# lemerleau/RAFFT

Measured on AMD Instinct MI355X. Metric: sequences/sec (whole node) on benchmark set, beam N=100; kcal/mol MAE vs CPU, higher is better.
Workload: dtype f32 FFT -> exact int counts, f64 scores, i32 dcal energies

## Files before the change

### rafft_amd/csrc/rafft_expand_small.hip

```cpp
#pragma once

template <int TL> struct SmLds {
    static constexpr int NL = 2 * TL;
    static constexpr int off_S = 0;
    static constexpr int off_pos = SM_SPAN + 8;
    static constexpr int off_br = off_pos + 2 * TL;
    static constexpr int off_pe = off_br + 4 * TL;
    static constexpr int off_psp = off_pe + 8 * (TL + 1);
    static constexpr int off_ck = (off_psp + 2 * (TL + 1) + 7) & ~7;
    static constexpr int off_val = off_ck + 8 * NL;
    static constexpr int per_team = (off_val + 8 * NL + 15) & ~15;
};
#define SM_GUARD 4608
static_assert(sizeof(SmallT) <= SM_GUARD, "energy tables must fit the guard area");
#define SM_WG_WAVES 4
template <int TL> constexpr int small_lds_bytes() { return SM_GUARD + SM_WG_WAVES * (64 / TL) * SmLds<TL>::per_team; }

#ifndef RAFFT_SMALL_WAVES
#define RAFFT_SMALL_WAVES 4
#endif

__device__ __forceinline__ uint32_t sm_shift(uint32_t x, int s)
{
    return s >= 0 ? (s < 32 ? x >> s : 0u) : (s > -32 ? x << -s : 0u);
}

template <int TL, bool PROD = false>
__global__ __launch_bounds__(64 * SM_WG_WAVES, RAFFT_SMALL_WAVES) void expand_small_kernel(Dev d, int cls_arg)
{
    const int cls = cls_arg & 0xFF;
    using LY = SmLds<TL>;
    constexpr int TPW = 64 / TL;
    extern __shared__ __align__(16) unsigned char lds_all[];
    {
        int *dst = (int *)lds_all;
        const int *src = (const int *)&d.T->s;
        for (int i = threadIdx.x; i < (int)(sizeof(SmallT) / 4); i += 64 * SM_WG_WAVES) dst[i] = src[i];
        __syncthreads();
    }
    const SmallT *T = (const SmallT *)lds_all;
    const BigT *B = &d.T->b;
    const int lane = threadIdx.x & 63, wv = threadIdx.x >> 6;
    const int tl = lane & (TL - 1), tq = lane / TL, tbase = tq * TL;
    const unsigned long long tmask = ((1ULL << TL) - 1ULL) << tbase;
    const unsigned long long lt_lane = (1ULL << lane) - 1ULL, lt_team = (1ULL << tbase) - 1ULL;
    const uint32_t TM = (uint32_t)((1ULL << TL) - 1ULL);
    unsigned char *lds = lds_all + SM_GUARD + (wv * TPW + tq) * LY::per_team;
    uint8_t *Sw = lds + LY::off_S;
    uint16_t *pos = (uint16_t *)(lds + LY::off_pos);
    uint32_t *brl = (uint32_t *)(lds + LY::off_br);
    int *pe_ext = (int *)(lds + LY::off_pe), *pe_ml = pe_ext + (TL + 1);
    uint16_t *psp = (uint16_t *)(lds + LY::off_psp);
    unsigned long long *ck = (unsigned long long *)(lds + LY::off_ck);
    double *val = (double *)(lds + LY::off_val);

    if (d.c->overflow) return;
    const unsigned n_items = d.c->n_work[cls].v;
    const unsigned gw = blockIdx.x * SM_WG_WAVES + wv, n_waves = gridDim.x * SM_WG_WAVES;
    if (gw == 0 && lane == 0) d.c->n_mat = 0;
    const int shard = gw & (NSHARD - 1);
    unsigned long long st_items = 0, st_n = 0, st_lags = 0, st_nbr = 0;
    unsigned int st_eval = 0, st_guess = 0, st_kguess = 0;
    const unsigned FETCH = n_items > 4u * TPW * n_waves ? (unsigned)d.fetch_bulk : 1u;
    unsigned fetch_base = 0, fetch_left = 0;
    const FetchPlan fplan = fetch_plan(d, n_items, FETCH * TPW, TPW);
    int fshard = (int)(gw & (NSHARD - 1));
    unsigned long long ffailed = 0;
    unsigned long long slab_base = 0; unsigned slab_left = 0;
    const bool dbg = !PROD && d.dbg.lag != nullptr;
    const double par_none = 0.0; (void)par_none;

    for (;;) {
        wave_sync();
        if (fetch_left == 0) {
            unsigned fcount = TPW;
            fetch_base = fetch_chunk(d, cls, fplan, fshard, ffailed, fcount);
            if (fetch_base == ~0u) break;
            fetch_left = fcount / TPW;
        }
        const unsigned item0 = fetch_base;
        fetch_base += TPW; fetch_left--;
        if (item0 >= n_items) { fetch_left = 0; continue; }
        const bool act = item0 + (unsigned)tq < n_items;
        const int nid = d.work[cls][act ? item0 + tq : item0];
        const NodeRec *nr = &d.nd[nid];
        const int n = nr->n, ci = nr->ci, cj = nr->cj, nbr = nr->nbr, L = nr->L, par_dcal = nr->pdcal;
        const uint16_t *posg = d.pos + nr->pos;
        const uint32_t *brg = d.br + nr->br;
        const uint8_t *codes = d.codes + nr->soff;
        const int sx0 = ci < 0 ? 0 : ci;
        const uint8_t *Sl = (const uint8_t *)Sw - sx0;
        const int m = 2 * n - 1;

        int myp = -1, c = 0;
        if (act && tl < n) {
            const int p = posg[tl];
            myp = p & 0x0FFF; c = p >> 12;
            pos[tl] = (uint16_t)myp;
            Sw[myp - sx0] = (uint8_t)c;
        }
        if (act && tl < nbr) {
            const uint32_t u = brg[tl];
            brl[tl] = u & 0x0FFF0FFFu;
            Sw[(int)(u & 0x0FFFu) - sx0] = (uint8_t)((u >> 12) & 0xFu);
            Sw[(int)((u >> 16) & 0x0FFFu) - sx0] = (uint8_t)(u >> 28);
        }
        if (act && ci >= 0 && tl < 2) { const int x = tl ? cj : ci; Sw[x - sx0] = codes[x]; }
        const uint32_t px_ = row16_or((uint32_t)((c + 3) & 3) << (2 * (tl & 15)));
        const unsigned long long p2 = (unsigned long long)(uint32_t)__shfl((int)px_, tbase + 15, 64) |
                                      (TL == 32 ? (unsigned long long)(uint32_t)__shfl((int)px_, tbase + 31, 64) << 32 : 0ULL);
        const unsigned long long bA = __ballot(c == 1), bC = __ballot(c == 2), bG = __ballot(c == 3), bU = __ballot(c == 4);
        const int pprev = __shfl_up(myp, 1, TL);
        const unsigned long long bg = __ballot(act && tl >= 1 && tl < n && myp - pprev == 1);
        const uint32_t mA = (uint32_t)(bA >> tbase) & TM, mC = (uint32_t)(bC >> tbase) & TM, mG = (uint32_t)(bG >> tbase) & TM,
                       mU = (uint32_t)(bU >> tbase) & TM, mg = (uint32_t)(bg >> tbase) & TM;
        const int rs = 32 - n;
        const uint32_t rA = __brev(mA) >> rs, rC = __brev(mC) >> rs, rG = __brev(mG) >> rs, rU = __brev(mU) >> rs, rg = __brev(mg) >> rs;
        wave_sync();
        double wgc = d.gc, wau = d.au, wgu = d.gu;
        asm volatile("" : "+v"(wgc), "+v"(wau), "+v"(wgu));

        int w_nb[2], w_mi[2], w_mj[2];
        double w_sc[2];
#pragma unroll
        for (int s = 0; s < 2; s++) {
            const int k = tl + s * TL;
            int mx_nb = 0, mx_i = 0, mx_j = 0;
            double mx_s = 0.0;
            if (act && k < m) {
                const int len = k < n ? k + 1 : 2 * n - k - 1;
                const int len2 = (len >> 1) + (len & 1);
                const int ip0 = k < n ? 0 : k - n + 1, jp0 = k < n ? k : n - 1;
                const int csure = len - 1 - d.min_hp;
                int lo = csure > 0 ? min((csure + 1) >> 1, len2) : 0, hi = len2;
                while (lo < hi) {
                    const int mid = (lo + hi) >> 1;
                    if ((int)pos[jp0 - mid] - (int)pos[ip0 + mid] > d.min_hp) lo = mid + 1; else hi = mid;
                }
                const int lim = lo;
                if (lim > 0) {
                    const int sft = n - 1 - k;
                    const uint32_t xA = sm_shift(rA, sft), xC = sm_shift(rC, sft), xG = sm_shift(rG, sft), xU = sm_shift(rU, sft);
                    const uint32_t pGC = d.gc != 0.0 ? ((mG & xC) | (mC & xG)) : 0u;
                    const uint32_t pAU = d.au != 0.0 ? ((mA & xU) | (mU & xA)) : 0u;
                    const uint32_t pGU = d.gu != 0.0 ? ((mG & xU) | (mU & xG)) : 0u;
                    const uint32_t cm = mg & sm_shift(rg, sft - 1) & ~(1u << ip0);
                    const uint32_t range = (lim >= 32 ? ~0u : ((1u << lim) - 1u)) << ip0;
                    uint32_t any = (pGC | pAU | pGU) & range;
                    double prev = 0.0;
                    int last_ip = -2, runlen = 0;
                    bool found = false;
                    while (any) {
                        const int ip = __ffs((int)any) - 1;
                        any &= any - 1;
                        const uint32_t bit = 1u << ip;
                        const double w8 = (pGC & bit) ? wgc : (pAU & bit) ? wau : wgu;
                        if (ip != last_ip + 1) { prev = 0.0; runlen = 0; }
                        double t = w8;
                        if (cm & bit) t = (prev + w8) * w8;
                        runlen++;
                        if (t >= mx_s) { mx_s = t; mx_nb = runlen; mx_i = ip; mx_j = k - ip; found = true; }
                        prev = t; last_ip = ip;
                    }
                    if (!found) { mx_i = ip0 + lim - 1; mx_j = k - mx_i; }
                }
            }
            w_nb[s] = mx_nb; w_mi[s] = mx_i; w_mj[s] = mx_j; w_sc[s] = mx_s;
        }

        int w_k[2] = {tl, tl + TL};
        if (!dbg) {
            const unsigned long long sb0 = __ballot(w_nb[0] > 0) & tmask, sb1 = __ballot(w_nb[1] > 0) & tmask;
            const int n0 = __popcll(sb0), nst = n0 + __popcll(sb1);
            uint32_t *sl = (uint32_t *)ck;
            if (w_nb[0] > 0) sl[__popcll(sb0 & lt_lane)] = (uint32_t)w_nb[0] | ((uint32_t)w_mi[0] << 8) | ((uint32_t)tl << 16);
            if (w_nb[1] > 0) sl[n0 + __popcll(sb1 & lt_lane)] = (uint32_t)w_nb[1] | ((uint32_t)w_mi[1] << 8) | ((uint32_t)(tl + TL) << 16);
            wave_sync();
#pragma unroll
            for (int s = 0; s < 2; s++) {
                const int idx = tl + s * TL;
                const uint32_t e = idx < nst ? sl[idx] : 0u;
                w_nb[s] = (int)(e & 255u); w_mi[s] = (int)((e >> 8) & 255u); w_k[s] = (int)(e >> 16); w_mj[s] = w_k[s] - w_mi[s];
            }
            wave_sync();
        }
        {
            int ve = 0, vm = 0, vs = 0;
            if (act && tl < nbr) {
                const uint32_t u = brl[tl];
                const int p = (int)(u & 0xffffu), q = (int)(u >> 16);
                const int tt = pair_type(Sl[p], Sl[q]);
                if (ci < 0) ve = e_stem(T, tt, p > 0 ? (int)Sl[p - 1] : -1, q < L - 1 ? (int)Sl[q + 1] : -1, true);
                vm = e_stem(T, tt, p > 0 ? (int)Sl[p - 1] : 0, q < L - 1 ? (int)Sl[q + 1] : 0, false);
                vs = q - p + 1;
            }
            int xe = ve, xm = vm, xs = vs;
#pragma unroll
            for (int o = 1; o < TL; o <<= 1) {
                const int ye = __shfl_up(xe, o, TL), ym = __shfl_up(xm, o, TL), ys = __shfl_up(xs, o, TL);
                if (tl >= o) { xe += ye; xm += ym; xs += ys; }
            }
            if (act && tl < nbr) { pe_ext[tl] = xe - ve; pe_ml[tl] = xm - vm; psp[tl] = (uint16_t)(xs - vs); }
            if (act && tl == (nbr > 0 ? nbr - 1 : 0)) {
                if (nbr > 0) { pe_ext[nbr] = xe; pe_ml[nbr] = xm; psp[nbr] = (uint16_t)xs; }
                else { pe_ext[0] = 0; pe_ml[0] = 0; psp[0] = 0; }
            }
        }
        wave_sync();
        const double par_e = dcal_to_energy(par_dcal);
        const BrPrefix pf{pe_ext, pe_ml, psp};
        int w_dd[2];
        bool w_keep[2];
        {
            const bool anystem = act && (w_nb[0] > 0 || w_nb[1] > 0);
            int e_old = 0, g_old = 0;
            if (anystem) {
                const BrList all_br{brl, 0, nbr, 0, 0, 0, 0, 0};
                e_old = loop_energy_pre(T, B, Sl, L, ci, cj, all_br, pf, g_old);
            }
#pragma unroll
            for (int s = 0; s < 2; s++) {
                w_dd[s] = 0; w_keep[s] = false;
                const int nb = w_nb[s];
                if (act && nb > 0) {
                    int g = g_old;
                    const int mi = w_mi[s], mj = w_mj[s];
                    const int a0 = pos[mi], b0 = pos[mj], ao = pos[mi - nb + 1], bo = pos[mj + nb - 1];
                    int lo, hi, lo_o, hi_o;
                    br_lower4(brl, nbr, a0, b0, ao, bo, lo, hi, lo_o, hi_o);
                    BrList outer{brl, 0, lo_o, hi_o, nbr, 1, ao, bo};
                    int e_new = loop_energy_pre(T, B, Sl, L, ci, cj, outer, pf, g);
                    BrList inner{brl, lo, hi, 0, 0, 0, 0, 0};
                    e_new += loop_energy_pre(T, B, Sl, L, a0, b0, inner, pf, g);
                    if (nb <= 16 && a0 - ao == nb - 1 && bo - b0 == nb - 1)
                        e_new += stem_stack_windows(T, (uint32_t)(p2 >> (2 * (mi - nb + 1))), (uint32_t)(p2 >> (2 * mj)), nb);
                    else {
                    int pa = a0, pb = b0, ty_in = pair_type(Sl[a0], Sl[b0]);
                    for (int t = 1; t < nb; t++) {
                        const int a = pos[mi - t], b = pos[mj + t];
                        const int ty = pair_type(Sl[a], Sl[b]);
                        if (pa == a + 1 && pb == b - 1)
                            e_new += T->stack[ty][rtype(ty_in)];
                        else {
                            const int lo2 = br_lower(brl, nbr, a), hi2 = br_lower(brl, nbr, b);
                            BrList mid{brl, lo2, lo, hi, hi2, 1, pa, pb};
                            e_new += loop_energy_pre(T, B, Sl, L, a, b, mid, pf, g);
                            lo = lo2; hi = hi2;
                        }
                        pa = a; pb = b; ty_in = ty;
                    }
                    }
                    const int ddc = e_new - e_old;
                    w_dd[s] = ddc;
                    const double dE = dcal_to_energy(par_dcal + ddc) - par_e;
                    w_keep[s] = dE < d.min_nrj;
                    st_eval++; st_guess += g ? 1 : 0; st_kguess += (g && w_keep[s]) ? 1 : 0;
                }
            }
        }
        double w_val[2] = {0.0, 0.0};
#pragma unroll
        for (int s = 0; s < 2; s++) {
            const int k = w_k[s];
            if ((w_keep[s] || dbg) && act && k < m) {
                const int sft = n - 1 - k;
                const uint32_t xU = sm_shift(rU, sft), xC = sm_shift(rC, sft);
                const double nAU = 2.0 * (double)__popc(mA & xU), nGC = 2.0 * (double)__popc(mG & xC), nGU = 2.0 * (double)__popc(mG & xU);
                const double raw = nAU * d.au + nGC * d.gc + nGU * d.gu;
                const int nk = k < m - 1 - k ? k : m - 1 - k;
                w_val[s] = raw / ((double)nk + 1.0);
            }
        }
        int w_rank[2] = {0, 0};
        if (dbg) {
#pragma unroll
            for (int s = 0; s < 2; s++) { const int k = tl + s * TL; if (act && k < m) val[k] = w_val[s]; }
            wave_sync();
#pragma unroll
            for (int s = 0; s < 2; s++) {
                const int k = tl + s * TL;
                if (act && k < m && tq == 0) {
                    int r = 0;
                    for (int y = 0; y < m; y++) { const double v = val[y]; r += (v > w_val[s] || (v == w_val[s] && y > k)) ? 1 : 0; }
                    w_rank[s] = r;
                    d.dbg.lag[r] = k; d.dbg.corval[r] = w_val[s];
                    d.dbg.nb[r] = w_nb[s]; d.dbg.mi[r] = w_mi[s]; d.dbg.mj[r] = w_mj[s]; d.dbg.score[r] = w_sc[s];
                    if (d.dbg.ddcal) d.dbg.ddcal[r] = w_nb[s] > 0 ? w_dd[s] : INT_MIN;
                }
            }
            if (lane == 0 && d.dbg.n_ranked) *d.dbg.n_ranked = m;
            wave_sync();
        }

        const unsigned long long kb0 = __ballot(w_keep[0]), kb1 = __ballot(w_keep[1]);
        const int nk0 = __popcll(kb0 & tmask), nkept = nk0 + __popcll(kb1 & tmask);
        const int toff = __popcll(kb0 & lt_team) + __popcll(kb1 & lt_team);
        const int tot = __popcll(kb0) + __popcll(kb1);
        const int slot[2] = {(int)__popcll(kb0 & tmask & lt_lane), nk0 + (int)__popcll(kb1 & tmask & lt_lane)};
        unsigned long long cbase = 0;
        int ovf = 0;
        if (lane == 0 && tot) {
            if ((unsigned)tot > slab_left) {
                const unsigned slab = d.cand_shard_cap >= 64u * (unsigned)d.cand_slab ? (unsigned)d.cand_slab : 16u;
                const unsigned want = (unsigned)tot > slab ? (unsigned)tot : slab;
                const unsigned long long b0 = atomicAdd(&d.c->cand[shard].v, (unsigned long long)want);
                if (b0 + want > d.cand_shard_cap) { atomicOr(&d.c->overflow, OVF_CAND); ovf = 1; slab_left = 0; }
                else { slab_base = (unsigned long long)shard * d.cand_shard_cap + b0; slab_left = want; }
            }
            if (!ovf) { cbase = slab_base; slab_base += tot; slab_left -= tot; }
        }
        cbase = __shfl(cbase, 0, 64);
        ovf = __shfl(ovf, 0, 64);
#pragma unroll
        for (int s = 0; s < 2; s++)
            if (w_keep[s]) {
                ck[slot[s]] = ((unsigned long long)((unsigned)w_dd[s] ^ 0x80000000u) << 32) | (unsigned)w_k[s];
                val[slot[s]] = w_val[s];
            }
        wave_sync();
        if (!ovf) {
#pragma unroll
            for (int s = 0; s < 2; s++)
                if (w_keep[s]) {
                    const int k = w_k[s];
                    const unsigned long long kx = ck[slot[s]];
                    int rank = 0;
                    for (int y = 0; y < nkept; y++) {
                        const unsigned long long ky = ck[y];
                        if ((ky >> 32) == (kx >> 32)) {
                            const int lagq = (int)(ky & 0xFFFFFFFFu);
                            const double qv = val[y];
                            rank += (lagq != k && (qv > w_val[s] || (qv == w_val[s] && lagq > k))) ? 1 : 0;
                        } else
                            rank += ky < kx ? 1 : 0;
                    }
                    const int mi = w_mi[s], mj = w_mj[s], nb = w_nb[s];
                    const int a0 = pos[mi], b0 = pos[mj], ao = pos[mi - nb + 1], bo = pos[mj + nb - 1];
                    uint64_t h1 = 0, h2 = 0;
                    if (a0 - ao == nb - 1 && bo - b0 == nb - 1) stem_hash(a0, b0, ao, bo, &h1, &h2);
                    else
                        for (int t = 0; t < nb; t++) {
                            uint64_t a, b;
                            pair_hash(pos[mi - t], pos[mj + t], &a, &b);
                            h1 += a; h2 += b;
                        }
                    Cand cd;
                    cd.ddcal = w_dd[s]; cd.mi = (uint16_t)mi; cd.mj = (uint16_t)mj; cd.nb = (uint16_t)nb;
                    { int c0, c1, c2, c3; br_lower4(brl, nbr, a0, b0, ao, bo, c0, c1, c2, c3); cd.set_cuts(c0, c1, c2, c3); }
                    cd.h1 = h1; cd.h2 = h2;
                    d.cand[cbase + toff + rank] = cd;
                    d.cslot[cbase + toff + rank] = 0ULL;
                    if (dbg && d.dbg.kept) d.dbg.kept[rank] = w_rank[s];
                }
        }
        if (act && tl == 0) {
            NodeRec *nw = &d.nd[nid];
            nw->cand = cbase + toff;
            nw->ncand = ovf ? 0 : nkept;
            if (dbg && d.dbg.n_ranked) d.dbg.n_ranked[1] = nkept;
            st_items++; st_n += n; st_lags += m; st_nbr += nbr;
        }
    }
    for (int o = 32; o > 0; o >>= 1) {
        st_items += __shfl_xor(st_items, o, 64); st_n += __shfl_xor(st_n, o, 64);
        st_lags += __shfl_xor(st_lags, o, 64); st_nbr += __shfl_xor(st_nbr, o, 64);
        st_eval += __shfl_xor(st_eval, o, 64); st_guess += __shfl_xor(st_guess, o, 64); st_kguess += __shfl_xor(st_kguess, o, 64);
    }
    if (lane == 0 && st_items) {
        Counters::StatLine *sl = &d.c->xstat[cls][gw & (NSHARD - 1)];
        atomicAdd(&sl->items, st_items);
        atomicAdd(&sl->n, st_n);
        atomicAdd(&sl->lags, st_lags);
        atomicAdd(&sl->nbr, st_nbr);
        if (T->lsb && st_eval) {
            atomicAdd(&sl->evals, (unsigned long long)st_eval);
            if (st_guess) atomicAdd(&sl->guessed, (unsigned long long)st_guess);
            if (st_kguess) atomicAdd(&sl->kept_guessed, (unsigned long long)st_kguess);
        }
    }
}
```

### rafft_amd/csrc/rafft_kernels.hip

```cpp
#include "rafft_kernels.h"


__device__ __forceinline__ float2 cmul(float2 a, float2 b)
{
    return make_float2(a.x * b.x - a.y * b.y, a.x * b.y + a.y * b.x);
}
__device__ __forceinline__ float2 cmulc(float2 a, float2 b)
{
    return make_float2(a.x * b.x + a.y * b.y, a.y * b.x - a.x * b.y);
}

__device__ __forceinline__ void pin(unsigned int &x) { asm volatile("" : "+v"(x)); }
__device__ __forceinline__ void pin(int &x) { asm volatile("" : "+v"(x)); }
__device__ __forceinline__ void pin(unsigned long long &x) { asm volatile("" : "+v"(x)); }
__device__ __forceinline__ void pin(ulonglong2 &x) { asm volatile("" : "+v"(x.x), "+v"(x.y)); }
__device__ __forceinline__ void pin(uint4 &x) { asm volatile("" : "+v"(x.x), "+v"(x.y), "+v"(x.z), "+v"(x.w)); }

template <int NT>
__device__ inline int block_exscan(int v, int *scratch, int *tot)
{
    const int lane = threadIdx.x & 63, wv = threadIdx.x >> 6;
    const int x = wave_incl_scan(v);
    if (NT == 64) {
        *tot = __builtin_amdgcn_readlane(x, 63);
// ... 508 lines not shown
        }
        if (selected) {
            int *hist = (int *)(lds + lay.offA + (LONGSEQ == 2 ? lay.szA - 2048 : nofft ? 8 * P + 8 * MASK_WORDS * ((nmax + 63) >> 6) : 9 * P));
            int *shs = hist + 256;
            auto ukey = [&](int i) -> unsigned long long {
                unsigned long long u = (unsigned long long)__double_as_longlong(keyv[i]);
                return (u >> 63) ? ~u : (u | 0x8000000000000000ULL);
            };
            unsigned long long prefix = 0;
            int kk = Kp;
            bool take_ge = false;
            int pass0 = 7;
            if (PROD) {
                if (NT > 64) {
                    if (tid < 3) shs[20 + tid] = 0;
                    ESYNC();
                    if ((tid & 63) == 0) { atomicAdd(&shs[20], c_hi); atomicAdd(&shs[21], c_lo); atomicOr(&shs[22], c_odd); }
                    ESYNC();
                    c_hi = shs[20]; c_lo = shs[21]; c_odd = shs[22];
                }
                if (!c_odd) {
                    const int c_zero = m - c_hi - c_lo;
                    int binc;
                    if (kk <= c_hi) { prefix = 0xC0ULL << 56; binc = c_hi; }
                    else if (kk <= c_hi + c_lo) { prefix = 0xBFULL << 56; kk -= c_hi; binc = c_lo; }
                    else { prefix = 0x80ULL << 56; kk -= c_hi + c_lo; binc = c_zero; }
                    pass0 = kk == binc ? -1 : 6;
                    take_ge = kk == binc;
                }
            }
            for (int pass = pass0; pass >= 0; pass--) {
                for (int i = tid; i < 256; i += NT) hist[i] = 0;
                ESYNC();
                const int sh_hi = 8 * (pass + 1);
                for (int i = tid; i < m; i += NT) {
                    const unsigned long long u = ukey(i);
                    if (pass == 7 || (u >> sh_hi) == (prefix >> sh_hi)) atomicAdd(&hist[(int)((u >> (8 * pass)) & 255ULL)], 1);
                }
                ESYNC();
                {
                    constexpr int BPT = NT >= 256 ? 1 : 256 / NT;
                    int hs[BPT], mine = 0;
#pragma unroll
                    for (int j = 0; j < BPT; j++) { const int bi = tid * BPT + j; hs[j] = bi < 256 ? hist[255 - bi] : 0; mine += hs[j]; }
                    int tot, ex = block_exscan<NT>(mine, shs, &tot);
#pragma unroll
                    for (int j = 0; j < BPT; j++) {
                        if (ex < kk && kk <= ex + hs[j] && hs[j] > 0) { shs[28] = 255 - (tid * BPT + j); shs[29] = kk - ex; shs[30] = hs[j]; }
                        ex += hs[j];
                    }
                    ESYNC();
                }
                prefix |= (unsigned long long)(unsigned)shs[28] << (8 * pass);
                kk = shs[29];
                const bool whole_bin = kk == shs[30];
                ESYNC();
                if (whole_bin) { take_ge = true; break; }
            }
            int outn = 0, tie_run = 0;
            for (int base = 0; base < P; base += NT) {
                const int i = P - 1 - (base + tid);
                unsigned long long u = 0;
                int tie = 0;
                if (i >= 0 && i < m) { u = ukey(i); tie = (u == prefix) ? 1 : 0; }
                int ttot = 0, tex = 0;
                if (!take_ge) tex = block_exscan_flag<NT>(tie, shs, &ttot);
                const int g = (i >= 0 && i < m) && (take_ge ? u >= prefix : (u > prefix || (tie && tie_run + tex < kk))) ? 1 : 0;
                int gtot, gex = block_exscan_flag<NT>(g, shs, &gtot);
                if (g) rk[outn + gex] = (uint16_t)i;
                outn += gtot; tie_run += ttot;
                ESYNC();
            }
            if (dbgrank) {
            int M2 = 2; while (M2 < Kp) M2 <<= 1;
            for (int i = Kp + tid; i < M2; i += NT) rk[i] = 0xFFFF;
            ESYNC();
            for (int k2 = 2; k2 <= M2; k2 <<= 1)
                for (int j = k2 >> 1; j > 0; j >>= 1) {
                    for (int i = tid; i < M2; i += NT) {
                        int ixj = i ^ j;
                        if (ixj > i) {
                            const uint16_t la = rk[i], lb = rk[ixj];
                            bool a_first;
                            if (la == 0xFFFF) a_first = false;
                            else if (lb == 0xFFFF) a_first = true;
                            else { const double va = keyv[la], vb = keyv[lb]; a_first = (va > vb) || (va == vb && la > lb); }
                            const bool up = (i & k2) == 0;
                            if (up ? !a_first : a_first) { rk[i] = lb; rk[ixj] = la; }
                        }
                    }
                    ESYNC();
                }
            }
            for (int r = tid; r < Kp; r += NT)
                if (dbg.lag) { dbg.lag[r] = rk[r]; dbg.corval[r] = keyv[rk[r]]; }
            if (tid == 0 && dbg.n_ranked) *dbg.n_ranked = Kp;
            ESYNC();
        } else {
        if (inplace)
            for (int k2 = 2; k2 <= P; k2 <<= 1) {
                for (int j = k2 >> 1; j > 0; j >>= 1) {
                    for (int i = tid; i < P; i += NT) {
                        int ixj = i ^ j;
                        if (ixj > i) {
                            double va = keyv[i], vb = keyv[ixj];
                            uint16_t la = lagk[i], lb = lagk[ixj];
                            bool a_first = (va > vb) || (va == vb && la > lb);
                            bool up = (i & k2) == 0;
                            if (up ? !a_first : a_first) {
                                keyv[i] = vb; keyv[ixj] = va;
                                lagk[i] = lb; lagk[ixj] = la;
                            }
                        }
                    }
                    ESYNC();
                }
            }
        for (int r = tid; r < Kp; r += NT) {
            rk[r] = inplace ? lagk[r] : (uint16_t)r;
            if (dbg.lag) { dbg.lag[r] = lagk[r]; dbg.corval[r] = keyv[r]; }
        }
        if (tid == 0 && dbg.n_ranked) *dbg.n_ranked = Kp;
        ESYNC();
        }

        const int C = (NT >= 256 && selected) ? max(1, min(8, NT / max(Kp, 1))) : 1;
        struct WsPart { double score; int nb, mi, mj, any; };
        WsPart *parts = (WsPart *)(lds + lay.offA + 8 * Pk);
        const bool ws_masks = PROD || (d.gc >= 0.0 && d.au >= 0.0 && d.gu >= 0.0 && !force_fft);
        if (ws_masks) {
            const int W = (n + 63) >> 6;
            unsigned long long *F = (unsigned long long *)(lds + lay.offA + (inplace ? 0 : 8 * Pk));
            unsigned long long *R = F + MASK_F_WORDS * W;
            parts = (WsPart *)(R + 5 * W);
            if (LONGSEQ != 2 && (!mw || inplace)) {
                build_masks<NT>(F, R, W, n, code_at, pos, tid);
                ESYNC();
            }
            const uint32_t *F32 = (const uint32_t *)F, *R32 = (const uint32_t *)R;
            const int W2 = 2 * W;
            double wgc = d.gc, wau = d.au, wgu = d.gu;
            asm volatile("" : "+v"(wgc), "+v"(wau), "+v"(wgu));
            auto win = [](const uint32_t *X, int start) -> uint32_t { const int q_ = start >> 5; return __builtin_amdgcn_alignbit(X[q_ + 1], X[q_], (uint32_t)(start & 31)); };
            for (int q = tid; q < Kp * C; q += NT) {
                const int r = q / C, c = q - r * C;
                const int lagp = rk[r];
                const int len = lagp < n ? lagp + 1 : 2 * n - lagp - 1;
                const int len2 = (len >> 1) + (len & 1);
                const int ip0 = lagp < n ? 0 : lagp - n + 1, jp0 = lagp < n ? lagp : n - 1;
                const int csure = len - 1 - d.min_hp;
                int lo = csure > 0 ? min((csure + 1) >> 1, len2) : 0, hi = len2;
                while (lo < hi) {
                    const int mid = (lo + hi) >> 1;
                    if ((int)pos[jp0 - mid] - (int)pos[ip0 + mid] > d.min_hp) lo = mid + 1; else hi = mid;
                }
                const int lim = lo;
                const int ca = (int)((long long)lim * c / C), ce = (int)((long long)lim * (c + 1) / C);
                const int rs0 = n - 1 - lagp + ip0;
                auto cells = [&](int k, uint32_t &pGC, uint32_t &pAU, uint32_t &pGU, uint32_t &cm) {
                    const int cs = ip0 + 32 * k, rs = rs0 + 32 * k;
                    const uint32_t fA = win(F32 + 0 * W2, cs), fC = win(F32 + 1 * W2, cs), fG = win(F32 + 2 * W2, cs), fU = win(F32 + 3 * W2, cs);
                    const uint32_t xA = win(R32 + 0 * W2, rs), xC = win(R32 + 1 * W2, rs), xG = win(R32 + 2 * W2, rs), xU = win(R32 + 3 * W2, rs);
                    pGC = d.gc != 0.0 ? ((fG & xC) | (fC & xG)) : 0u;
                    pAU = d.au != 0.0 ? ((fA & xU) | (fU & xA)) : 0u;
                    pGU = d.gu != 0.0 ? ((fG & xU) | (fU & xG)) : 0u;
                    cm = win(F32 + 4 * W2, cs) & win(R32 + 4 * W2, rs);
                    if (k == 0) cm &= ~1u;
                };
                auto span = [](int lo_, int hi_, int cb) -> uint32_t {
                    uint32_t m_ = ~0u;
                    if (lo_ > cb) m_ &= ~0u << (lo_ - cb);
                    if (hi_ < cb + 32) m_ &= (1u << (hi_ - cb)) - 1u;
                    return m_;
                };
                double mx_s = 0.0, prev = 0.0;
                int mx_nb = 0, mx_c = 0, last_c = -2, runlen = 0, mx_i = 0, mx_j = 0;
                if (ce > ca) {
                    int z = ca;
                    if (ca > 0) {
                        for (int kz = (ca - 1) >> 5;; kz--) {
                            const int cb = kz << 5;
                            uint32_t pGC, pAU, pGU, cm;
                            cells(kz, pGC, pAU, pGU, cm);
                            const uint32_t zeros = ~(pGC | pAU | pGU) & span(0, ca, cb);
                            if (zeros) { z = cb + 32 - __clz((int)zeros); break; }
                            if (cb == 0) { z = 0; break; }
                        }
                    }
                    for (int k = z >> 5; k <= (ce - 1) >> 5; k++) {
                        const int cb = k << 5;
                        uint32_t pGC, pAU, pGU, cm;
                        cells(k, pGC, pAU, pGU, cm);
                        uint32_t any = (pGC | pAU | pGU) & span(z, ce, cb);
                        while (any) {
                            const int bi = __ffs((int)any) - 1;
                            any &= any - 1u;
                            const int cc = cb + bi;
                            const double w8 = ((pGC >> bi) & 1u) ? wgc : ((pAU >> bi) & 1u) ? wau : wgu;
                            if (cc != last_c + 1) { prev = 0.0; runlen = 0; }
                            double t = w8;
                            if ((cm >> bi) & 1u) t = (prev + w8) * w8;
                            runlen++;
                            if ((C == 1 || cc >= ca) && t >= mx_s) { mx_s = t; mx_nb = runlen; mx_c = cc; }
                            prev = t; last_c = cc;
                        }
                    }
                    if (mx_nb == 0) mx_c = ce - 1;
                    mx_i = ip0 + mx_c; mx_j = lagp - mx_i;
                }
                if (C == 1) {
                    wnb[r] = (uint16_t)mx_nb; wmi[r] = (uint16_t)mx_i;
                    if (dbg.nb) { dbg.nb[r] = mx_nb; dbg.mi[r] = mx_i; dbg.mj[r] = mx_j; dbg.score[r] = mx_s; }
                } else {
                    WsPart wp; wp.score = mx_s; wp.nb = mx_nb; wp.mi = mx_i; wp.mj = mx_j; wp.any = ce > ca ? 1 : 0;
                    parts[q] = wp;
                }
            }
            if (C > 1) {
                ESYNC();
                for (int r = tid; r < Kp; r += NT) {
                    double mx_s = 0.0;
                    int mx_nb = 0, mx_i = 0, mx_j = 0;
                    for (int c = 0; c < C; c++) {
                        const WsPart wp = parts[r * C + c];
                        if (wp.any && wp.score >= mx_s) { mx_s = wp.score; mx_nb = wp.nb; mx_i = wp.mi; mx_j = wp.mj; }
                    }
                    wnb[r] = (uint16_t)mx_nb; wmi[r] = (uint16_t)mx_i;
                    if (dbg.nb) { dbg.nb[r] = mx_nb; dbg.mi[r] = mx_i; dbg.mj[r] = mx_j; dbg.score[r] = mx_s; }
                }
            }
        } else {
            for (int q = tid; q < Kp * C; q += NT) {
                const int r = q / C, c = q - r * C;
                const int lagp = rk[r];
                const int len = lagp < n ? lagp + 1 : 2 * n - lagp - 1;
                const int len2 = (len >> 1) + (len & 1);
                const int a = (int)((long long)len2 * c / C), e = (int)((long long)len2 * (c + 1) / C);
                const int ip0 = lagp < n ? 0 : lagp - n + 1, jp0 = lagp < n ? lagp : n - 1;
                int z = a;
                while (z > 0 && wtab[code_at(ip0 + z - 1) * 5 + code_at(jp0 - (z - 1))] != 0.0) z--;
                double prev = 0.0, mx_s = 0.0;
                int tmp = 0, mx_nb = 0, mx_i = 0, mx_j = 0, any = 0;
                for (int i = z; i < e; i++) {
                    const int ip = ip0 + i, jp = jp0 - i;
                    double t = wtab[code_at(ip) * 5 + code_at(jp)];
                    if (i > 0 && (int)pos[ip] - (int)pos[ip - 1] == 1 && (int)pos[jp + 1] - (int)pos[jp] == 1)
                        t = (prev + t) * t;
                    tmp = (t == 0.0) ? 0 : tmp + 1;
                    if (i >= a && t >= mx_s && (int)pos[jp] - (int)pos[ip] > d.min_hp) {
                        mx_s = t; mx_nb = tmp; mx_i = ip; mx_j = jp; any = 1;
                    }
                    prev = t;
                }
                if (C == 1) {
                    wnb[r] = (uint16_t)mx_nb; wmi[r] = (uint16_t)mx_i;
                    if (dbg.nb) { dbg.nb[r] = mx_nb; dbg.mi[r] = mx_i; dbg.mj[r] = mx_j; dbg.score[r] = mx_s; }
                } else {
                    WsPart w; w.score = mx_s; w.nb = mx_nb; w.mi = mx_i; w.mj = mx_j; w.any = any;
                    parts[q] = w;
                }
            }
            if (C > 1) {
                ESYNC();
                for (int r = tid; r < Kp; r += NT) {
                    double mx_s = 0.0;
                    int mx_nb = 0, mx_i = 0, mx_j = 0;
                    for (int c = 0; c < C; c++) {
                        const WsPart w = parts[r * C + c];
                        if (w.any && w.score >= mx_s) { mx_s = w.score; mx_nb = w.nb; mx_i = w.mi; mx_j = w.mj; }
                    }
                    wnb[r] = (uint16_t)mx_nb; wmi[r] = (uint16_t)mx_i;
                    if (dbg.nb) { dbg.nb[r] = mx_nb; dbg.mi[r] = mx_i; dbg.mj[r] = mx_j; dbg.score[r] = mx_s; }
                }
            }
        }
        ESYNC();

        const double par_e = dcal_to_energy(par_dcal);
        int *pe_ext = (int *)(lds + lay.offA + (inplace ? 0 : 8 * Pk));
        int *pe_ml = pe_ext + (nbr + 1);
        uint16_t *psp = (uint16_t *)(pe_ml + (nbr + 1));
        if (tid < 64) {
            int c_e = 0, c_m = 0, c_s = 0;
            for (int base = 0; base < nbr; base += 64) {
                const int i = base + tid;
                int ve = 0, vm = 0, vs = 0;
                if (i < nbr) {
                    const uint32_t u = brl[i];
                    const int p = (int)(u & 0xffffu), q = (int)(u >> 16);
                    const int tt = pair_type(Sl[p], Sl[q]);
                    if (ci < 0) ve = e_stem(T, tt, p > 0 ? (int)Sl[p - 1] : -1, q < L - 1 ? (int)Sl[q + 1] : -1, true);
                    vm = e_stem(T, tt, p > 0 ? (int)Sl[p - 1] : 0, q < L - 1 ? (int)Sl[q + 1] : 0, false);
                    vs = q - p + 1;
                }
                const int xe = wave_incl_scan(ve), xm = wave_incl_scan(vm), xs = wave_incl_scan(vs);
                if (i < nbr) { pe_ext[i] = c_e + xe - ve; pe_ml[i] = c_m + xm - vm; psp[i] = (uint16_t)(c_s + xs - vs); }
                c_e += __builtin_amdgcn_readlane(xe, 63); c_m += __builtin_amdgcn_readlane(xm, 63); c_s += __builtin_amdgcn_readlane(xs, 63);
            }
            if (tid == 0) { pe_ext[nbr] = c_e; pe_ml[nbr] = c_m; psp[nbr] = (uint16_t)c_s; }
        }
        ESYNC();
        const BrPrefix pf{pe_ext, pe_ml, psp};
        const BrList all_br{brl, 0, nbr, 0, 0, 0, 0, 0};
        int g_old = 0;
        const int e_old = loop_energy_pre(T, B, Sl, L, ci, cj, all_br, pf, g_old);
        int nst = 0;
        for (int base = 0; base < Kp; base += NT) {
            const int r = base + tid;
            const int f = (r < Kp && wnb[r] > 0) ? 1 : 0;
            if (r < Kp) keep[r] = 0;
            int tot, ex = block_exscan_flag<NT>(f, misc + 16, &tot);
            if (f) widx[nst + ex] = (uint16_t)r;
            nst += tot;
        }
        ESYNC();
        for (int si = tid; si < nst; si += NT) {
            const int r = widx[si];
            const int nb = wnb[r];
            {
                int g = g_old;
                const int mi = wmi[r], mj = (int)rk[r] - mi;
                const int a0 = pos[mi], b0 = pos[mj], ao = pos[mi - nb + 1], bo = pos[mj + nb - 1];
                int lo, hi, lo_o, hi_o;
                br_lower4(brl, nbr, a0, b0, ao, bo, lo, hi, lo_o, hi_o);
                BrList outer{brl, 0, lo_o, hi_o, nbr, 1, ao, bo};
                int e_new = loop_energy_pre(T, B, Sl, L, ci, cj, outer, pf, g);
                BrList inner{brl, lo, hi, 0, 0, 0, 0, 0};
                e_new += loop_energy_pre(T, B, Sl, L, a0, b0, inner, pf, g);
                if (CODE_LDS && nb <= 16 && a0 - ao == nb - 1 && bo - b0 == nb - 1)
                    e_new += stem_stack_windows(T, strand_window(P2, mi - nb + 1), strand_window(P2, mj), nb);
                else {
                int pa = a0, pb = b0, ty_in = pair_type(Sl[a0], Sl[b0]);
                for (int t = 1; t < nb; t++) {
                    const int a = pos[mi - t], b = pos[mj + t];
                    const int ty = pair_type(Sl[a], Sl[b]);
                    if (pa == a + 1 && pb == b - 1)
                        e_new += T->stack[ty][rtype(ty_in)];
                    else {
                        const int lo2 = br_lower(brl, nbr, a), hi2 = br_lower(brl, nbr, b);
                        BrList mid{brl, lo2, lo, hi, hi2, 1, pa, pb};
                        e_new += loop_energy_pre(T, B, Sl, L, a, b, mid, pf, g);
                        lo = lo2; hi = hi2;
                    }
                    pa = a; pb = b; ty_in = ty;
                }
                }
                const int ddc = e_new - e_old;
                dd[r] = ddc;
                const double dE = dcal_to_energy(par_dcal + ddc) - par_e;
                keep[r] = (uint16_t)(((dE < d.min_nrj) ? 1 : 0) | (g ? 2 : 0) | 4);
                if (dbg.ddcal) dbg.ddcal[r] = ddc;
            }
        }
        if (dbg.ddcal) for (int r = tid; r < Kp; r += NT) if (wnb[r] == 0) dbg.ddcal[r] = INT_MIN;
        ESYNC();

        int nkept = 0;
        if constexpr (NT == 64) {
            unsigned long long *kbs = (unsigned long long *)&misc[8];
            for (int base = 0; base < Kp; base += 64) {
                const int r = base + tid;
                const int kf = (r < Kp) ? keep[r] : 0;
                const unsigned long long bal = __ballot((kf & 1) != 0);
                if (T->lsb) {
                    const int ne = __popcll(__ballot((kf & 4) != 0)), ng = __popcll(__ballot((kf & 6) == 6)), nk = __popcll(__ballot((kf & 3) == 3));
                    if (tid == 0) { atomicAdd(&misc[24], ne); if (ng) atomicAdd(&misc[25], ng); if (nk) atomicAdd(&misc[26], nk); }
                }
                if (tid == 0) kbs[base >> 6] = bal;
                if (kf & 1) keep[nkept + (int)__builtin_amdgcn_mbcnt_hi((unsigned)(bal >> 32), __builtin_amdgcn_mbcnt_lo((unsigned)bal, 0u))] = (uint16_t)r;
                nkept += __popcll(bal);
            }
            st_items++; st_n += n; st_lags += Kp; st_nbr += nbr;
            unsigned long long cbase = 0;
            int ovf_i = 0;
            if (nkept) {
                unsigned long long b0 = 0;
                const bool fresh = (unsigned)nkept > slab_left;
                const unsigned slab = d.cand_shard_cap >= 64u * (unsigned)d.cand_slab ? (unsigned)d.cand_slab : 16u;
                const unsigned want = (unsigned)nkept > slab ? (unsigned)nkept : slab;
                if (fresh) {
                    if (tid == 0) b0 = atomicAdd(&d.c->cand[shard].v, (unsigned long long)want);
                    b0 = ((unsigned long long)(unsigned)__builtin_amdgcn_readfirstlane((int)(b0 >> 32)) << 32) | (unsigned)__builtin_amdgcn_readfirstlane((int)b0);
                    if (b0 + want > d.cand_shard_cap) { if (tid == 0) atomicOr(&d.c->overflow, OVF_CAND); ovf_i = 1; slab_left = 0; }
                    else { slab_base = (unsigned long long)shard * d.cand_shard_cap + b0; slab_left = want; }
                }
                if (!ovf_i) { cbase = slab_base; slab_base += nkept; slab_left -= nkept; }
            }
            wave_sync();
            if (nkept && !ovf_i)
            for (int x = tid; x < nkept; x += 64) {
                {
                    const int r = keep[x];
                    const int my = dd[r];
                    int rank = 0;
                    for (int b2 = 0; b2 < Kp; b2 += 64) {
                        const unsigned long long mv = kbs[b2 >> 6];
                        unsigned long long m = ((unsigned long long)(unsigned)__builtin_amdgcn_readfirstlane((int)(mv >> 32)) << 32) | (unsigned)__builtin_amdgcn_readfirstlane((int)mv);
                        while (m) {
                            const int y = b2 + __ffsll((long long)m) - 1;
                            m &= m - 1;
                            const int dy = dd[y];
                            if (dy < my) rank++;
                            else if (dy == my && y != r) {
                                if (inplace) rank += y < r ? 1 : 0;
                                else {
                                    const int lagq = rk[y], lagr = rk[r];
                                    const double qv = keyv[lagq], myv = keyv[lagr];
                                    rank += ((qv > myv) || (qv == myv && lagq > lagr)) ? 1 : 0;
                                }
                            }
                        }
                    }
                    const int mi = wmi[r], mj = (int)rk[r] - mi, nb = wnb[r];
                    const int a0 = pos[mi], b0 = pos[mj], ao = pos[mi - nb + 1], bo = pos[mj + nb - 1];
                    uint64_t h1 = 0, h2 = 0;
                    if (a0 - ao == nb - 1 && bo - b0 == nb - 1) stem_hash(a0, b0, ao, bo, &h1, &h2);
                    else
                        for (int t = 0; t < nb; t++) {
                            uint64_t a, b;
                            pair_hash(pos[mi - t], pos[mj + t], &a, &b);
                            h1 += a; h2 += b;
                        }
                    Cand cd;
                    cd.ddcal = my; cd.mi = (uint16_t)mi; cd.mj = (uint16_t)mj; cd.nb = (uint16_t)nb;
                    { int c0, c1, c2, c3; br_lower4(brl, nbr, a0, b0, ao, bo, c0, c1, c2, c3); cd.set_cuts(c0, c1, c2, c3); }
                    cd.h1 = h1; cd.h2 = h2;
                    d.cand[cbase + rank] = cd; d.cslot[cbase + rank] = 0ULL;
                    if (dbg.kept) dbg.kept[rank] = r;
                }
            }
            if (tid == 0) {
                d.nd[nid].cand = cbase;
                d.nd[nid].ncand = ovf_i ? 0 : nkept;
                if (dbg.n_ranked) dbg.n_ranked[1] = nkept;
            }
        } else {
        {
            int *wave_tot = misc + 16;
            const int lane = tid & 63, wv = tid >> 6;
            for (int base = 0; base < Kp; base += NT) {
                const int r = base + tid;
                const int kf = (r < Kp) ? keep[r] : 0;
                const int f = kf & 1;
                ESYNC();
                const unsigned long long bal = __ballot(f != 0);
                if (T->lsb) {
                    const int ne = __popcll(__ballot((kf & 4) != 0)), ng = __popcll(__ballot((kf & 6) == 6)), nk = __popcll(__ballot((kf & 3) == 3));
                    if (lane == 0) { atomicAdd(&misc[24], ne); if (ng) atomicAdd(&misc[25], ng); if (nk) atomicAdd(&misc[26], nk); }
                }
                int pre = __popcll(bal & ((1ULL << lane) - 1));
                if (NT > 64) {
                    if (lane == 0) wave_tot[wv] = __popcll(bal);
                    ESYNC();
                    int tot = 0;
                    for (int w = 0; w < NT / 64; w++) { if (w < wv) pre += wave_tot[w]; tot += wave_tot[w]; }
                    if (f) keep[nkept + pre] = (uint16_t)r;
                    nkept += tot;
                    ESYNC();
                } else {
                    if (f) keep[nkept + pre] = (uint16_t)r;
                    nkept += __popcll(bal);
                }
            }
            ESYNC();
        }
        if (tid == 0) {
            unsigned long long base = 0;
            misc[2] = 0;
            if (nkept) {
                if ((unsigned)nkept > slab_left) {
                    const unsigned slab = d.cand_shard_cap >= 64u * (unsigned)d.cand_slab ? (unsigned)d.cand_slab : 16u;
                    const unsigned want = (unsigned)nkept > slab ? (unsigned)nkept : slab;
                    unsigned long long b0 = atomicAdd(&d.c->cand[shard].v, (unsigned long long)want);
                    if (b0 + want > d.cand_shard_cap) { atomicOr(&d.c->overflow, OVF_CAND); misc[2] = 1; slab_left = 0; }
                    else { slab_base = (unsigned long long)shard * d.cand_shard_cap + b0; slab_left = want; }
                }
                if (!misc[2]) { base = slab_base; slab_base += nkept; slab_left -= nkept; }
            }
            *(unsigned long long *)&misc[4] = base;
            st_items++; st_n += n; st_lags += Kp; st_nbr += nbr;
        }
        ESYNC();
        const unsigned long long cbase = *(unsigned long long *)&misc[4];
        const bool ovf = misc[2] != 0;
        if (!ovf) {
            unsigned long long *ck = (unsigned long long *)(lds + lay.offA + (inplace ? 0 : 8 * Pk));
            for (int x = tid; x < nkept; x += NT) {
                const int r = keep[x];
                ck[x] = ((unsigned long long)((unsigned)dd[r] ^ 0x80000000u) << 32) | (unsigned)r;
            }
            ESYNC();
            for (int x = tid; x < nkept; x += NT) {
                const unsigned long long kx = ck[x];
                const int r = (int)(kx & 0xFFFFFFFFu);
                const int my = dd[r];
                int rank = 0;
                if (inplace) {
                    for (int y = 0; y < nkept; y++) rank += ck[y] < kx ? 1 : 0;
                } else {
                    const int lagr = rk[r];
                    const double myv = keyv[lagr];
                    for (int y = 0; y < nkept; y++) {
                        const unsigned long long ky = ck[y];
                        if ((ky >> 32) == (kx >> 32)) {
                            const int q = (int)(ky & 0xFFFFFFFFu), lagq = rk[q];
                            const double qv = keyv[lagq];
                            rank += (q != r && ((qv > myv) || (qv == myv && lagq > lagr))) ? 1 : 0;
                        } else
                            rank += ky < kx ? 1 : 0;
                    }
                }
                int mi = wmi[r], mj = (int)rk[r] - mi, nb = wnb[r];
                const int a0 = pos[mi], b0 = pos[mj], ao = pos[mi - nb + 1], bo = pos[mj + nb - 1];
                uint64_t h1 = 0, h2 = 0;
                if (a0 - ao == nb - 1 && bo - b0 == nb - 1) stem_hash(a0, b0, ao, bo, &h1, &h2);
                else
                    for (int t = 0; t < nb; t++) {
                        uint64_t a, b;
                        pair_hash(pos[mi - t], pos[mj + t], &a, &b);
                        h1 += a; h2 += b;
                    }
                Cand cd;
                cd.ddcal = my; cd.mi = (uint16_t)mi; cd.mj = (uint16_t)mj; cd.nb = (uint16_t)nb;
                { int c0, c1, c2, c3; br_lower4(brl, nbr, a0, b0, ao, bo, c0, c1, c2, c3); cd.set_cuts(c0, c1, c2, c3); }
                cd.h1 = h1; cd.h2 = h2;
                d.cand[cbase + rank] = cd; d.cslot[cbase + rank] = 0ULL;
                if (dbg.kept) dbg.kept[rank] = r;
            }
        }
        if (tid == 0) {
            d.nd[nid].cand = cbase;
            d.nd[nid].ncand = ovf ? 0 : nkept;
            if (dbg.n_ranked) dbg.n_ranked[1] = nkept;
        }
        }
    }
    if (tid == 0 && st_items) {
        Counters::StatLine *sl = &d.c->xstat[cls][gteam & (NSHARD - 1)];
        atomicAdd(&sl->items, st_items);
        atomicAdd(&sl->n, st_n);
        atomicAdd(&sl->lags, st_lags);
        atomicAdd(&sl->nbr, st_nbr);
    }
    if (tid == 0 && misc[24]) {
        Counters::StatLine *sl = &d.c->xstat[cls][gteam & (NSHARD - 1)];
        atomicAdd(&sl->evals, (unsigned long long)(unsigned)misc[24]);
        if (misc[25]) atomicAdd(&sl->guessed, (unsigned long long)(unsigned)misc[25]);
        if (misc[26]) atomicAdd(&sl->kept_guessed, (unsigned long long)(unsigned)misc[26]);
    }
}

#include "rafft_expand_small.hip"


__device__ inline bool seen_lookup(const uint64_t *tab, uint32_t cap, uint64_t h1, uint64_t h2, uint32_t &free_sl)
{
    const uint32_t mask = cap - 1;
    uint32_t sl = (uint32_t)h1 & mask;
    const ulonglong2 *t2 = (const ulonglong2 *)tab;
    for (;;) {
        const uint32_t s1 = (sl + 1) & mask, s2 = (sl + 2) & mask, s3 = (sl + 3) & mask;
        ulonglong2 e0 = t2[sl], e1 = t2[s1], e2 = t2[s2], e3 = t2[s3];
        pin(e0); pin(e1); pin(e2); pin(e3);
        if (e0.x == 0) { free_sl = sl; return false; }
        if (e0.x == h1 && e0.y == h2) return true;
        if (e1.x == 0) { free_sl = s1; return false; }
        if (e1.x == h1 && e1.y == h2) return true;
        if (e2.x == 0) { free_sl = s2; return false; }
        if (e2.x == h1 && e2.y == h2) return true;
        if (e3.x == 0) { free_sl = s3; return false; }
        if (e3.x == h1 && e3.y == h2) return true;
        sl = (sl + 4) & mask;
    }
}
__device__ inline void seen_insert_at(uint64_t *tab, uint32_t cap, uint64_t h1, uint64_t h2, uint32_t sl)
{
    const uint32_t mask = cap - 1;
    for (;;) {
        unsigned long long old = atomicCAS((unsigned long long *)&tab[2 * (uint64_t)sl], 0ULL, (unsigned long long)h1);
        if (old == 0) { tab[2 * (uint64_t)sl + 1] = h2; return; }
        if (old == h1 && tab[2 * (uint64_t)sl + 1] == h2) return;
        sl = (sl + 1) & mask;
    }
}
__device__ inline bool seen_insert_new(uint64_t *tab, uint32_t cap, uint64_t h1, uint64_t h2)
{
    uint32_t mask = cap - 1, sl = (uint32_t)h1 & mask;
    for (;;) {
        unsigned long long old = atomicCAS((unsigned long long *)&tab[2 * (uint64_t)sl], 0ULL, (unsigned long long)h1);
        if (old == 0) { tab[2 * (uint64_t)sl + 1] = h2; return true; }
        if (old == h1 && tab[2 * (uint64_t)sl + 1] == h2) return false;
        sl = (sl + 1) & mask;
    }
}
__device__ inline void seen_insert(uint64_t *tab, uint32_t cap, uint64_t h1, uint64_t h2)
{
    uint32_t mask = cap - 1, sl = (uint32_t)h1 & mask;
    for (;;) {
        unsigned long long old = atomicCAS((unsigned long long *)&tab[2 * (uint64_t)sl], 0ULL, (unsigned long long)h1);
        if (old == 0) { tab[2 * (uint64_t)sl + 1] = h2; return; }
        if (old == h1 && tab[2 * (uint64_t)sl + 1] == h2) return;
        sl = (sl + 1) & mask;
    }
}


template <int NT>
__device__ inline void seen_rehash(const uint64_t *stab, uint32_t scap, uint64_t *ntab, uint32_t ncap, int tid)
{
    const ulonglong2 *src = (const ulonglong2 *)stab;
    const uint32_t mask = ncap - 1;
    for (uint32_t base = 0; base < scap; base += NT * 4) {
        ulonglong2 e[4];
        unsigned long long old[4];
#pragma unroll
        for (int u = 0; u < 4; u++) { const uint32_t i = base + (uint32_t)u * NT + (uint32_t)tid; e[u] = i < scap ? src[i] : make_ulonglong2(0ULL, 0ULL); }
#pragma unroll
        for (int u = 0; u < 4; u++) { old[u] = 1; if (e[u].x) old[u] = atomicCAS((unsigned long long *)&ntab[2 * (uint64_t)((uint32_t)e[u].x & mask)], 0ULL, (unsigned long long)e[u].x); }
#pragma unroll
        for (int u = 0; u < 4; u++)
            if (e[u].x) {
                if (old[u] == 0) ntab[2 * (uint64_t)((uint32_t)e[u].x & mask) + 1] = e[u].y;
                else seen_insert(ntab, ncap, e[u].x, e[u].y);
            }
    }
}

struct ParentInfo {
    unsigned long long total, cur;
    unsigned long long h1, h2;
    int dcal0, flag;
    int sid, nprod;
    unsigned long long prod;
    int rl0, nrl;
};
static_assert(sizeof(ParentInfo) == 64, "ParentInfo layout");

__device__ __forceinline__ unsigned long long sat_mul(unsigned long long a, unsigned long long b)
{
    const unsigned long long lim = 1ULL << 62;
    if (a == 0 || b == 0) return 0;
    return (a > lim / b) ? lim : a * b;
}

template <int BS_NT>
__global__ __launch_bounds__(BS_NT, BS_NT == 256 ? 5 : 1) void beam_step_kernel(Dev d, int sort_cap)
{
    extern __shared__ __align__(16) unsigned char lds[];
    const size_t r0 = max((size_t)8 * (size_t)sort_cap, (size_t)24 * BS_NT);
    unsigned long long *skey = (unsigned long long *)lds;
    unsigned long long *wk_h1 = (unsigned long long *)lds;
    unsigned long long *wk_h2 = wk_h1 + BS_NT;
    unsigned int *wk_tab = (unsigned int *)(wk_h2 + BS_NT);
// ... 1001 lines not shown
```

Baseline: 533,200.

## Split stem energy evaluation into half-work items across lanes with DPP pairing

Each candidate stem's energy delta evaluation is split into two work items, the outer loop and the inner loop plus stack terms. Consecutive lanes take one half each and their results are summed with a DPP quad-permute swap. The parent loop energy becomes item zero, computed in the same pass instead of serially by every thread. This aims to cut lane imbalance and serial loop_energy_pre latency, at the cost of extra LDS staging, more passes when there are many stems, and added barriers.

After: 516,200. 3.2% lower.

```diff
diff --git a/rafft_amd/csrc/rafft_expand_small.hip b/rafft_amd/csrc/rafft_expand_small.hip
--- a/rafft_amd/csrc/rafft_expand_small.hip
+++ b/rafft_amd/csrc/rafft_expand_small.hip
@@ -169,10 +169,12 @@
         }
 
         int w_k[2] = {tl, tl + TL};
+        uint32_t *sl = (uint32_t *)ck;
+        int nst;
         if (!dbg) {
             const unsigned long long sb0 = __ballot(w_nb[0] > 0) & tmask, sb1 = __ballot(w_nb[1] > 0) & tmask;
-            const int n0 = __popcll(sb0), nst = n0 + __popcll(sb1);
-            uint32_t *sl = (uint32_t *)ck;
+            const int n0 = __popcll(sb0);
+            nst = n0 + __popcll(sb1);
             if (w_nb[0] > 0) sl[__popcll(sb0 & lt_lane)] = (uint32_t)w_nb[0] | ((uint32_t)w_mi[0] << 8) | ((uint32_t)tl << 16);
             if (w_nb[1] > 0) sl[n0 + __popcll(sb1 & lt_lane)] = (uint32_t)w_nb[1] | ((uint32_t)w_mi[1] << 8) | ((uint32_t)(tl + TL) << 16);
             wave_sync();
@@ -182,8 +184,12 @@
                 const uint32_t e = idx < nst ? sl[idx] : 0u;
                 w_nb[s] = (int)(e & 255u); w_mi[s] = (int)((e >> 8) & 255u); w_k[s] = (int)(e >> 16); w_mj[s] = w_k[s] - w_mi[s];
             }
-            wave_sync();
-        }
+        } else {
+            nst = act ? m : 0;
+#pragma unroll
+            for (int s = 0; s < 2; s++) sl[tl + s * TL] = (uint32_t)w_nb[s] | ((uint32_t)w_mi[s] << 8) | ((uint32_t)(tl + s * TL) << 16);
+        }
+        wave_sync();
         {
             int ve = 0, vm = 0, vs = 0;
             if (act && tl < nbr) {
@@ -212,51 +218,68 @@
         int w_dd[2];
         bool w_keep[2];
         {
-            const bool anystem = act && (w_nb[0] > 0 || w_nb[1] > 0);
+            int *res = (int *)val;
+            const int nitems = nst > 0 ? 2 * nst + 2 : 0;
             int e_old = 0, g_old = 0;
-            if (anystem) {
-                const BrList all_br{brl, 0, nbr, 0, 0, 0, 0, 0};
-                e_old = loop_energy_pre(T, B, Sl, L, ci, cj, all_br, pf, g_old);
-            }
-#pragma unroll
-            for (int s = 0; s < 2; s++) {
-                w_dd[s] = 0; w_keep[s] = false;
-                const int nb = w_nb[s];
-                if (act && nb > 0) {
-                    int g = g_old;
-                    const int mi = w_mi[s], mj = w_mj[s];
-                    const int a0 = pos[mi], b0 = pos[mj], ao = pos[mi - nb + 1], bo = pos[mj + nb - 1];
-                    int lo, hi, lo_o, hi_o;
-                    br_lower4(brl, nbr, a0, b0, ao, bo, lo, hi, lo_o, hi_o);
-                    BrList outer{brl, 0, lo_o, hi_o, nbr, 1, ao, bo};
-                    int e_new = loop_energy_pre(T, B, Sl, L, ci, cj, outer, pf, g);
-                    BrList inner{brl, lo, hi, 0, 0, 0, 0, 0};
-                    e_new += loop_energy_pre(T, B, Sl, L, a0, b0, inner, pf, g);
+            for (int ps = 0; __ballot(ps * TL < nitems) != 0ULL; ps++) {
+                const int it = ps * TL + tl;
+                const int si = (it >> 1) - 1;
+                const bool in_half = (it & 1) != 0;
+                const uint32_t se = (si >= 0 && si < nst) ? sl[si] : 0u;
+                const int nb = (int)(se & 255u);
+                const bool stem = nb > 0;
+                int e = 0, g = 0;
+                if (stem || (it == 0 && nitems > 0)) {
+                    int lci = ci, lcj = cj, mi = 0, mj = 0, a0 = 0, b0 = 0, ao = 0, bo = 0, lo = 0, hi = 0;
+                    BrList bl{brl, 0, nbr, 0, 0, 0, 0, 0};
+                    if (stem) {
+                        mi = (int)((se >> 8) & 255u); mj = (int)(se >> 16) - mi;
+                        a0 = pos[mi]; b0 = pos[mj]; ao = pos[mi - nb + 1]; bo = pos[mj + nb - 1];
+                        int lo_o, hi_o;
+                        br_lower4(brl, nbr, a0, b0, ao, bo, lo, hi, lo_o, hi_o);
+                        if (in_half) { lci = a0; lcj = b0; bl = BrList{brl, lo, hi, 0, 0, 0, 0, 0}; }
+                        else bl = BrList{brl, 0, lo_o, hi_o, nbr, 1, ao, bo};
+                    }
+                    e = loop_energy_pre(T, B, Sl, L, lci, lcj, bl, pf, g);
+                    if (stem && in_half) {
                     if (nb <= 16 && a0 - ao == nb - 1 && bo - b0 == nb - 1)
-                        e_new += stem_stack_windows(T, (uint32_t)(p2 >> (2 * (mi - nb + 1))), (uint32_t)(p2 >> (2 * mj)), nb);
+                        e += stem_stack_windows(T, (uint32_t)(p2 >> (2 * (mi - nb + 1))), (uint32_t)(p2 >> (2 * mj)), nb);
                     else {
                     int pa = a0, pb = b0, ty_in = pair_type(Sl[a0], Sl[b0]);
                     for (int t = 1; t < nb; t++) {
                         const int a = pos[mi - t], b = pos[mj + t];
                         const int ty = pair_type(Sl[a], Sl[b]);
                         if (pa == a + 1 && pb == b - 1)
-                            e_new += T->stack[ty][rtype(ty_in)];
+                            e += T->stack[ty][rtype(ty_in)];
                         else {
                             const int lo2 = br_lower(brl, nbr, a), hi2 = br_lower(brl, nbr, b);
                             BrList mid{brl, lo2, lo, hi, hi2, 1, pa, pb};
-                            e_new += loop_energy_pre(T, B, Sl, L, a, b, mid, pf, g);
+                            e += loop_energy_pre(T, B, Sl, L, a, b, mid, pf, g);
                             lo = lo2; hi = hi2;
                         }
                         pa = a; pb = b; ty_in = ty;
                     }
                     }
-                    const int ddc = e_new - e_old;
+                    }
+                }
+                if (ps == 0) { e_old = __shfl(e, tbase, 64); g_old = __shfl(g, tbase, 64); }
+                const int e_new = e + __builtin_amdgcn_update_dpp(0, e, 0xB1, 0xF, 0xF, true);
+                const int g2 = g | __builtin_amdgcn_update_dpp(0, g, 0xB1, 0xF, 0xF, true) | g_old;
+                if (stem && !in_half) { res[si] = e_new - e_old; res[LY::NL + si] = g2; }
+            }
+            wave_sync();
+#pragma unroll
+            for (int s = 0; s < 2; s++) {
+                w_dd[s] = 0; w_keep[s] = false;
+                if (act && w_nb[s] > 0) {
+                    const int ddc = res[tl + s * TL], g = res[LY::NL + tl + s * TL];
                     w_dd[s] = ddc;
                     const double dE = dcal_to_energy(par_dcal + ddc) - par_e;
                     w_keep[s] = dE < d.min_nrj;
                     st_eval++; st_guess += g ? 1 : 0; st_kguess += (g && w_keep[s]) ? 1 : 0;
                 }
             }
+            wave_sync();
         }
         double w_val[2] = {0.0, 0.0};
 #pragma unroll
diff --git a/rafft_amd/csrc/rafft_kernels.hip b/rafft_amd/csrc/rafft_kernels.hip
--- a/rafft_amd/csrc/rafft_kernels.hip
+++ b/rafft_amd/csrc/rafft_kernels.hip
@@ -834,8 +834,6 @@
         ESYNC();
         const BrPrefix pf{pe_ext, pe_ml, psp};
         const BrList all_br{brl, 0, nbr, 0, 0, 0, 0, 0};
-        int g_old = 0;
-        const int e_old = loop_energy_pre(T, B, Sl, L, ci, cj, all_br, pf, g_old);
         int nst = 0;
         for (int base = 0; base < Kp; base += NT) {
             const int r = base + tid;
@@ -846,41 +844,63 @@
             nst += tot;
         }
         ESYNC();
-        for (int si = tid; si < nst; si += NT) {
-            const int r = widx[si];
-            const int nb = wnb[r];
-            {
-                int g = g_old;
-                const int mi = wmi[r], mj = (int)rk[r] - mi;
-                const int a0 = pos[mi], b0 = pos[mj], ao = pos[mi - nb + 1], bo = pos[mj + nb - 1];
-                int lo, hi, lo_o, hi_o;
-                br_lower4(brl, nbr, a0, b0, ao, bo, lo, hi, lo_o, hi_o);
-                BrList outer{brl, 0, lo_o, hi_o, nbr, 1, ao, bo};
-                int e_new = loop_energy_pre(T, B, Sl, L, ci, cj, outer, pf, g);
-                BrList inner{brl, lo, hi, 0, 0, 0, 0, 0};
-                e_new += loop_energy_pre(T, B, Sl, L, a0, b0, inner, pf, g);
+        int e_old = 0, g_old = 0;
+        const int nitems = 2 * nst + 2;
+        for (int base = 0; base < nitems; base += NT) {
+            const int it = base + tid;
+            const int si = (it >> 1) - 1;
+            const bool in_half = (it & 1) != 0, stem = si >= 0 && si < nst;
+            int e = 0, g = 0, r = 0;
+            if (stem || it == 0) {
+                int lci = ci, lcj = cj, nb = 0, mi = 0, mj = 0, a0 = 0, b0 = 0, ao = 0, bo = 0, lo = 0, hi = 0;
+                BrList bl = all_br;
+                if (stem) {
+                    r = widx[si];
+                    nb = wnb[r];
+                    mi = wmi[r]; mj = (int)rk[r] - mi;
+                    a0 = pos[mi]; b0 = pos[mj]; ao = pos[mi - nb + 1]; bo = pos[mj + nb - 1];
+                    int lo_o, hi_o;
+                    br_lower4(brl, nbr, a0, b0, ao, bo, lo, hi, lo_o, hi_o);
+                    if (in_half) { lci = a0; lcj = b0; bl = BrList{brl, lo, hi, 0, 0, 0, 0, 0}; }
+                    else bl = BrList{brl, 0, lo_o, hi_o, nbr, 1, ao, bo};
+                }
+                e = loop_energy_pre(T, B, Sl, L, lci, lcj, bl, pf, g);
+                if (stem && in_half) {
                 if (CODE_LDS && nb <= 16 && a0 - ao == nb - 1 && bo - b0 == nb - 1)
-                    e_new += stem_stack_windows(T, strand_window(P2, mi - nb + 1), strand_window(P2, mj), nb);
+                    e += stem_stack_windows(T, strand_window(P2, mi - nb + 1), strand_window(P2, mj), nb);
                 else {
                 int pa = a0, pb = b0, ty_in = pair_type(Sl[a0], Sl[b0]);
                 for (int t = 1; t < nb; t++) {
                     const int a = pos[mi - t], b = pos[mj + t];
                     const int ty = pair_type(Sl[a], Sl[b]);
                     if (pa == a + 1 && pb == b - 1)
-                        e_new += T->stack[ty][rtype(ty_in)];
+                        e += T->stack[ty][rtype(ty_in)];
                     else {
                         const int lo2 = br_lower(brl, nbr, a), hi2 = br_lower(brl, nbr, b);
                         BrList mid{brl, lo2, lo, hi, hi2, 1, pa, pb};
-                        e_new += loop_energy_pre(T, B, Sl, L, a, b, mid, pf, g);
+                        e += loop_energy_pre(T, B, Sl, L, a, b, mid, pf, g);
                         lo = lo2; hi = hi2;
                     }
                     pa = a; pb = b; ty_in = ty;
                 }
                 }
+                }
+            }
+            if (base == 0) {
+                if (NT == 64) { e_old = __builtin_amdgcn_readfirstlane(e); g_old = __builtin_amdgcn_readfirstlane(g); }
+                else {
+                    if (tid == 0) { misc[0] = e; misc[1] = g; }
+                    ESYNC();
+                    e_old = misc[0]; g_old = misc[1];
+                }
+            }
+            const int e_new = e + __builtin_amdgcn_update_dpp(0, e, 0xB1, 0xF, 0xF, true);
+            const int g2 = g | __builtin_amdgcn_update_dpp(0, g, 0xB1, 0xF, 0xF, true) | g_old;
+            if (stem && !in_half) {
                 const int ddc = e_new - e_old;
                 dd[r] = ddc;
                 const double dE = dcal_to_energy(par_dcal + ddc) - par_e;
-                keep[r] = (uint16_t)(((dE < d.min_nrj) ? 1 : 0) | (g ? 2 : 0) | 4);
+                keep[r] = (uint16_t)(((dE < d.min_nrj) ? 1 : 0) | (g2 ? 2 : 0) | 4);
                 if (dbg.ddcal) dbg.ddcal[r] = ddc;
             }
         }
```
